# MarkFzp/Deep-Whole-Body-Control

Measured on AMD Instinct MI355X. Metric: env-steps/sec whole node, widowGo1 4096-env PPO, higher is better.
Workload: dtype f32

## Files before the change

### __graft_entry__.py

```python
import os
import subprocess
import sys

ROOT = os.path.dirname(os.path.abspath(__file__))
PKG = os.path.join(ROOT, "deep-whole-body-control_amd")
CSRC = os.path.join(PKG, "csrc")
LIB = os.path.join(PKG, "wbc_amd", "libwbc_amd.so")
SOURCES = ["wbc_sim.hip", "wbc_step_kernel.hip", "wbc_gae_kernel.hip", "wbc_policy_kernel.hip", "wbc_ppo_kernel.hip", "wbc_hist_kernel.hip", "wbc_hist_train_kernel.hip", "wbc_arm_kernel.hip", "wbc_proximity_kernel.hip", "wbc_estimator_kernel.hip", "wbc_mpc_kernel.hip", "wbc_footstep_kernel.hip", "wbc_contact_kernel.hip", "wbc_legctl_kernel.hip", "wbc_attitude_kernel.hip", "wbc_ground_kernel.hip", "wbc_slip_kernel.hip", "wbc_terrain_kernel.hip"]
for p in (PKG, os.path.join(ROOT, "oracle")):
    if p not in sys.path:
        sys.path.insert(0, p)


def _stale(target, deps):
    if not os.path.exists(target):
        return True
    t = os.path.getmtime(target)
    return any(os.path.getmtime(d) > t for d in deps)


COMMON_FLAGS = ["--offload-arch=gfx950", "-O3", "-std=c++17", "-fPIC", "-Wno-unused-result", "-fno-slp-vectorize"]
EXTRA_FLAGS = {"wbc_step_kernel.hip": ["-mllvm", "-disable-machine-licm"]}
HEADERS = ("wbc_device.h", "wbc_mlp.h", "wbc_chain_fwd.h", "wbc_ppo_chain.h", "wbc_stream_guard.h", "wbc_track.h", "wbc_stats.h", "wbc_tree.h", "wbc_urdf.h", "wbc_delassus.h", "wbc_proximity.h", "wbc_estimator.h", "wbc_mpc.h", "wbc_footstep.h", "wbc_contact.h", "wbc_legctl.h", "wbc_attitude.h", "wbc_ground.h", "wbc_slip.h")


def compile_objects(force: bool = False, extra=(), objdir=None, jobs: int = 4):
    from concurrent.futures import ThreadPoolExecutor
    objdir = objdir or os.path.join(ROOT, "build", "obj")
    os.makedirs(objdir, exist_ok=True)
    hipcc = os.environ.get("HIPCC", "/opt/rocm/bin/hipcc")
    hdrs = [os.path.join(CSRC, h) for h in HEADERS] + [os.path.join(ROOT, "include", "wbc_sim.h"), os.path.abspath(__file__)]
    todo, objs = [], []
    for src in SOURCES:
        obj = os.path.join(objdir, src.replace(".hip", ".o"))
        objs.append(obj)
        if force or _stale(obj, [os.path.join(CSRC, src)] + hdrs):
            todo.append([hipcc] + COMMON_FLAGS + EXTRA_FLAGS.get(src, []) + list(extra) + ["-c", os.path.join(CSRC, src), "-o", obj])
    with ThreadPoolExecutor(max_workers=jobs) as ex:
        list(ex.map(subprocess.check_call, todo))
    return objs


def build_product(force: bool = False) -> None:
    srcs = [os.path.join(CSRC, s) for s in SOURCES]
    deps = srcs + [os.path.join(CSRC, h) for h in HEADERS] + [os.path.join(ROOT, "include", "wbc_sim.h"), os.path.abspath(__file__)]
    if force or _stale(LIB, deps):
        objs = compile_objects(force)
        hipcc = os.environ.get("HIPCC", "/opt/rocm/bin/hipcc")
        subprocess.check_call([hipcc, "--offload-arch=gfx950", "-shared", "-fPIC", "-o", LIB] + objs)
    import wbc_amd
    from wbc_amd import native
    L = native.lib()
    missing = [s for s in native.EXPORTED_SYMBOLS if not hasattr(L, s)]
    if missing:
        raise RuntimeError(f"libwbc_amd.so lacks symbols: {missing}")


def build(force: bool = False) -> None:
    build_product(force)
    try:
        import oracle
        oracle.build(force)
    except Exception as e:
        print(f"[build] WARNING: the CPU oracle (test infrastructure) did not build: {e!r}", file=sys.stderr)


def smoke() -> None:
    import numpy as np
    import torch
    assert torch.cuda.is_available(), "smoke() needs a ROCm GPU"
    build()
    from oracle import OracleSim, default_curriculum
    from wbc_amd import abi
    from wbc_amd.config import WidowGo1RoughCfg, WidowGo1RoughCfgPPO, class_to_dict
    from wbc_amd.envs import WidowGo1
    from wbc_amd.rsl_rl.runners import OnPolicyRunner
    cfg = WidowGo1RoughCfg()
    cfg.env.num_envs = 64
    cfg.terrain.mesh_type = "plane"
    env = WidowGo1(cfg, sim_device="cuda:0", seed=3)
    o = OracleSim(env.wmodel, env.tcfg, 64, seed=3, precision="f64")
    o.set_curriculum(default_curriculum(cfg, 0))
    env.sim.reset_all()
    torch.cuda.synchronize()
    for name in abi.TENSOR_IDS:
        if name not in ("OBS_BUF",):
# ... 21 lines not shown
```

### deep-whole-body-control_amd/csrc/wbc_hist_kernel.hip

```cpp
#include <hip/hip_runtime.h>
#include "wbc_stream_guard.h"
#include <stdint.h>

#define H_T 10
#define H_NP 76
#define H_OBS 860
#define H_OFF 100
#define H_C1 30
#define H_C2 20
#define H_C3 10
#define H_OUT 20
#define H_ROWS 24
#define H_THREADS 256

struct HistParams { const float *enc_w, *enc_b, *c1_w, *c1_b, *c2_w, *c2_b, *lin_w, *lin_b; };

static __device__ __forceinline__ float elu1(float x) { return x > 0.f ? x : __expf(x) - 1.f; }

typedef float f32x4h __attribute__((ext_vector_type(4)));

static __device__ __forceinline__ void hist_latent_body(const HistParams& P, const float* __restrict__ obs, float* __restrict__ out, int rows) {
  __shared__ float b_enc[H_C1], b_c1[H_C2], b_c2[H_C3];
  __shared__ __attribute__((aligned(8))) float w_c2[H_C3][H_C2 * 2 + 2];
  __shared__ float w_lin[H_OUT][H_C1], b_lin[H_OUT];
// ... 77 lines not shown
      }
    }
    __syncthreads();
    for (int e = tid; e < H_ROWS * 3 * H_C3; e += H_THREADS) {
      const int rr = e / (3 * H_C3), rem = e - rr * (3 * H_C3), l = rem / H_C3, co = rem - l * H_C3;
      float acc = b_c2[co];
      const float* wr = w_c2[co];
#pragma unroll 4
      for (int ci = 0; ci < H_C2; ++ci) acc += h2[rr][l][ci] * wr[ci * 2] + h2[rr][l + 1][ci] * wr[ci * 2 + 1];
      h3[rr][co * 3 + l] = elu1(acc);
    }
    __syncthreads();
    for (int e = tid; e < H_ROWS * H_OUT; e += H_THREADS) {
      const int rr = e / H_OUT, j = e - rr * H_OUT;
      if (row0 + rr < rows) {
        float acc = b_lin[j];
#pragma unroll 6
        for (int i = 0; i < H_C1; ++i) acc += h3[rr][i] * w_lin[j][i];
        out[(size_t)(row0 + rr) * H_OUT + j] = elu1(acc);
      }
    }
  }
}

extern "C" __global__ void __launch_bounds__(H_THREADS, 3) wbc_hist_latent_kernel(HistParams P, const float* __restrict__ obs, float* __restrict__ out,
                                                                              int rows) {
  hist_latent_body(P, obs, out, rows);
}
extern "C" __global__ void __launch_bounds__(H_THREADS, 2) wbc_hist_latent_small_kernel(HistParams P, const float* __restrict__ obs,
                                                                                    float* __restrict__ out, int rows) {
  hist_latent_body(P, obs, out, rows);
}

extern "C" int wbc_hist_latent(const void* const* params, const float* obs, float* out, int rows, void* stream) {
  StreamDeviceGuard sdg(stream);
  if (!params || !obs || !out || rows <= 0) return -1;
  HistParams P;
  const float** dst = reinterpret_cast<const float**>(&P);
  for (int i = 0; i < 8; ++i) { if (!params[i]) return -1; dst[i] = static_cast<const float*>(params[i]); }
  const int ngroups = (rows + H_ROWS - 1) / H_ROWS;
  if (ngroups <= 512) hipLaunchKernelGGL(wbc_hist_latent_small_kernel, dim3(ngroups), dim3(H_THREADS), 0, (hipStream_t)stream, P, obs, out, rows);
  else hipLaunchKernelGGL(wbc_hist_latent_kernel, dim3(768), dim3(H_THREADS), 0, (hipStream_t)stream, P, obs, out, rows);
  return hipGetLastError() == hipSuccess ? 0 : -2;
}
```

### deep-whole-body-control_amd/wbc_amd/native.py

```python
from __future__ import annotations

import ctypes as C
import os

from . import abi

_HERE = os.path.dirname(os.path.abspath(__file__))
LIB_PATH = os.environ.get("WBC_AMD_LIB") or os.path.join(_HERE, "libwbc_amd.so")
_lib = None

c_void, c_int, c_f32p = C.c_void_p, C.c_int, C.c_void_p


class WbcError(RuntimeError):
    pass


def lib():
    global _lib
    if _lib is None:
        import torch
        if not os.path.exists(LIB_PATH):
            raise WbcError(f"{LIB_PATH} not found: build the HIP extension first "
                           f"(python -c 'import __graft_entry__ as g; g.build()')")
# ... 1 lines not shown
        L.wbc_last_error.restype = C.c_char_p
        L.wbc_sim_arena_bytes.restype = C.c_size_t
        L.wbc_sim_arena_bytes.argtypes = [c_int]
        L.wbc_sim_create.argtypes = [C.POINTER(abi.WbcModel), C.POINTER(abi.WbcTaskCfg), c_int, c_int, C.c_uint64,
                                     c_void, C.c_size_t, C.POINTER(c_void)]
        L.wbc_sim_destroy.argtypes = [c_void]
        L.wbc_sim_get_tensor.argtypes = [c_void, c_int, C.POINTER(c_void), C.POINTER(C.c_int64), C.POINTER(c_int), C.POINTER(c_int)]
        L.wbc_sim_set_env_params.argtypes = [c_void] + [c_void] * 10
        L.wbc_sim_set_heightfield.argtypes = [c_void, c_void, c_int, c_int] + [C.c_float] * 5
        L.wbc_sim_set_curriculum.argtypes = [c_void, C.POINTER(abi.WbcCurriculum)]
        L.wbc_sim_step.argtypes = [c_void, c_void, c_void]
        L.wbc_sim_step_to.argtypes = [c_void, c_void, c_void, c_void]
        L.wbc_sim_step_rollout.argtypes = [c_void, c_void, c_void, c_void, C.c_float, c_void, c_void, c_void]
        L.wbc_get_heights.argtypes = [c_void, c_int, c_void, c_int, c_void, c_void, c_int, c_int, C.c_float, C.c_float, C.c_float, c_void, c_int, c_int, c_void]
        L.wbc_sim_reset_all.argtypes = [c_void, c_void]
        L.wbc_sim_set_dof_forces.argtypes = [c_void, c_void, c_void]
        L.wbc_sim_simulate.argtypes = [c_void, c_void]
        L.wbc_sim_set_root_state.argtypes = [c_void, c_void, c_void]
        L.wbc_sim_set_dof_state.argtypes = [c_void, c_void, c_void]
        L.wbc_sim_set_root_state_indexed.argtypes = [c_void, c_void, c_void, c_int, c_void]
        L.wbc_sim_set_dof_state_indexed.argtypes = [c_void, c_void, c_void, c_int, c_void]
        for fn in ("wbc_sim_refresh_dof_state", "wbc_sim_refresh_root_state", "wbc_sim_refresh_net_contact_force",
                   "wbc_sim_refresh_force_sensor"):
            getattr(L, fn).argtypes = [c_void]
        L.wbc_sim_refresh_rigid_body_state.argtypes = [c_void, c_void]
        L.wbc_sim_get_step_counter.argtypes = [c_void, C.POINTER(C.c_int64)]
        L.wbc_sim_set_step_counter.argtypes = [c_void, C.c_int64]
        L.wbc_gae_compute.argtypes = [c_void] * 7 + [c_int, c_int, C.c_float, C.c_float, c_void]
        L.wbc_gae_normalize.argtypes = [c_void, c_void, C.c_int64, c_void]
        L.wbc_gae_workspace_doubles.argtypes = [c_int]
        L.wbc_abi_sizes.argtypes = [C.POINTER(c_int)]
        L.wbc_tensor_spec.argtypes = [c_int, C.POINTER(C.c_int64), C.POINTER(c_int), C.POINTER(c_int)]
        L.wbc_hist_latent.argtypes = [c_void, c_void, c_void, c_int, c_void]
        L.wbc_sim_arm_dynamics.argtypes = [c_void, c_void, c_void, c_void, c_void, c_void, c_void]
        L.wbc_sim_body_dynamics.argtypes = [c_void, c_void, c_void, c_void]
        L.wbc_sim_inverse_dynamics.argtypes = [c_void, c_void, c_void, c_void, c_void]
        L.wbc_sim_mass_solve.argtypes = [c_void, c_void, C.c_int64, c_int, c_void, c_int, c_void]
        L.wbc_sim_forward_dynamics.argtypes = [c_void, c_void, c_void, c_int, c_void]
        L.wbc_sim_body_accelerations.argtypes = [c_void, c_void, c_void, c_void]
        L.wbc_sim_centroidal.argtypes = [c_void] * 7
        L.wbc_sim_coriolis.argtypes = [c_void] * 5
        L.wbc_sim_momentum_observer.argtypes = [c_void, c_void, C.c_float, C.c_float, c_int, c_void, c_void]
        L.wbc_sim_proximity_pair_count.argtypes = [c_void]
        L.wbc_sim_proximity_pairs.argtypes = [c_void, c_void]
        L.wbc_sim_proximity.argtypes = [c_void] * 6 + [c_int, c_void]
        L.wbc_sim_leg_odometry.argtypes = [c_void, C.POINTER(abi.WbcEstimatorCfg)] + [c_void] * 8 + [c_int] + [c_void] * 6
        L.wbc_sim_footstep_plan.argtypes = [c_void, C.POINTER(abi.WbcFootstepCfg)] + [c_void] * 8 + [c_int] + [c_void] * 10
        L.wbc_sim_contact_detect.argtypes = ([c_void, C.POINTER(abi.WbcContactCfg)] + [c_void] * 4 + [c_int] + [c_void] * 4 + [c_int] + [c_void] * 2 +
                                             [c_int] + [c_void] * 8)
        L.wbc_sim_leg_control.argtypes = ([c_void, C.POINTER(abi.WbcLegControlCfg)] + [c_void] * 9 + [c_int, c_void, c_int, c_void, c_int] +
                                          [c_void] * 2 + [c_int] + [c_void] * 5)
        L.wbc_sim_attitude_filter.argtypes = [c_void, C.POINTER(abi.WbcAttitudeCfg)] + [c_void] * 5 + [c_int] + [c_void] * 2 + [c_int] + [c_void] * 8
        L.wbc_sim_ground_estimate.argtypes = [c_void, C.POINTER(abi.WbcGroundCfg)] + [c_void] * 6 + [c_int] * 2 + [c_void] * 9
        L.wbc_sim_slip_detect.argtypes = [c_void, C.POINTER(abi.WbcSlipCfg)] + [c_void] * 9 + [c_int] + [c_void] * 12
        L.wbc_sim_centroidal_mpc.argtypes = [c_void, C.POINTER(abi.WbcMpcCfg)] + [c_void] * 4 + [c_int] + [c_void] * 3 + [c_int] + [c_void] * 8
        L.wbc_sim_centroidal_mpc_workspace_floats.argtypes = [c_int]
        L.wbc_sim_centroidal_mpc_workspace_floats.restype = C.c_size_t
        L.wbc_sim_inverse_dynamics_derivatives.argtypes =[c_void, c_void, c_void, c_void, c_int, c_void]
        L.wbc_sim_forward_dynamics_derivatives_workspace_floats.argtypes = [c_int]
        L.wbc_sim_forward_dynamics_derivatives_workspace_floats.restype = C.c_size_t
        L.wbc_sim_forward_dynamics_derivatives.argtypes = [c_void, c_void, c_void, c_void, c_void, c_void, c_int, c_void, c_void]
        L.wbc_sim_inverse_dynamics_regressor.argtypes = [c_void, c_void, c_int, c_void, c_void, c_int, c_void]
        L.wbc_sim_forward_dynamics_sensitivity.argtypes = [c_void, c_void, c_int, c_void, c_void, c_void, c_void, c_int, c_void]
        L.wbc_sim_identification_accumulate.argtypes = [c_void, c_void, c_int, c_void, c_void, c_void, C.c_float] + [c_void] * 4 + [c_int, c_void]
        L.wbc_sim_identification_solve.argtypes = [c_void, c_int] + [c_void] * 5 + [C.c_float] + [c_void] * 6
        L.wbc_sim_constrained_dynamics_workspace_floats.argtypes = [c_int, c_int]
# ... 48 lines not shown
        L.wbc_asset_opts_default.restype = None
        L.wbc_asset_load_urdf.argtypes = [C.c_char_p, C.POINTER(abi.WbcAssetOpts), c_void, C.POINTER(c_void)]
        L.wbc_asset_dof_properties_ex.argtypes = [c_void, C.POINTER(abi.WbcDofProps)]
        L.wbc_asset_find_rigid_body.argtypes = L.wbc_asset_find_dof.argtypes = [c_void, C.c_char_p]
        L.wbc_asset_force_sensor_bodies.argtypes = [c_void, C.POINTER(C.c_int32)]
        L.wbc_ppo_sq_partials_offset.argtypes = [c_int]
        L.wbc_ppo_sq_partials_offset.restype = C.c_size_t
        L.wbc_ppo_clip_adam.argtypes = [c_void] * 4 + [C.c_float] * 7 + [c_void, c_void, c_void]
        L.wbc_ppo_clip_adam_packed.argtypes = [c_void] * 4 + [C.c_float] * 7 + [c_void, c_void, c_void, c_int, c_void]
        L.wbc_hist_train_grad.argtypes = [c_void, c_void, c_void, c_void, c_int, c_void, c_void, c_void]
        L.wbc_hist_train_workspace_floats.restype = C.c_size_t
        L.wbc_hist_clip_adam.argtypes = [c_void] * 4 + [C.c_float] * 7 + [c_int, c_void, c_void]
        L.wbc_priv_latent.argtypes = [c_void, c_void, c_void, c_int, c_void]
        L.wbc_ppo_workspace_floats.argtypes = [c_int]
        L.wbc_ppo_workspace_floats.restype = C.c_size_t
        _lib = L
    return _lib


EXPORTED_SYMBOLS = [
    "wbc_last_error", "wbc_sim_arena_bytes", "wbc_sim_create", "wbc_sim_destroy", "wbc_sim_get_tensor",
    "wbc_sim_set_env_params", "wbc_sim_set_heightfield", "wbc_sim_set_curriculum", "wbc_sim_step", "wbc_sim_step_to", "wbc_sim_step_rollout", "wbc_get_heights", "wbc_sim_reset_all",
    "wbc_sim_set_dof_forces", "wbc_sim_simulate", "wbc_sim_set_root_state", "wbc_sim_set_dof_state",
    "wbc_sim_set_root_state_indexed", "wbc_sim_set_dof_state_indexed", "wbc_sim_refresh_dof_state",
    "wbc_sim_refresh_root_state", "wbc_sim_refresh_net_contact_force", "wbc_sim_refresh_force_sensor",
    "wbc_sim_refresh_rigid_body_state", "wbc_sim_get_step_counter", "wbc_sim_set_step_counter", "wbc_gae_compute",
    "wbc_gae_normalize", "wbc_gae_workspace_doubles", "wbc_abi_sizes", "wbc_sim_episode_stats", "wbc_rollout_store", "wbc_hist_latent", "wbc_sim_arm_dynamics", "wbc_sim_body_dynamics", "wbc_sim_inverse_dynamics", "wbc_sim_mass_solve", "wbc_sim_forward_dynamics", "wbc_sim_body_accelerations", "wbc_sim_constrained_dynamics", "wbc_sim_constrained_dynamics_workspace_floats", "wbc_sim_constrained_dynamics_derivatives", "wbc_sim_constrained_dynamics_derivatives_workspace_floats", "wbc_sim_impulse_dynamics", "wbc_sim_impulse_dynamics_workspace_floats", "wbc_sim_inverse_kinematics", "wbc_sim_task_inverse_dynamics", "wbc_sim_task_inverse_dynamics_workspace_floats", "wbc_sim_task_inverse_dynamics_qp", "wbc_sim_task_inverse_dynamics_qp_workspace_floats", "wbc_sim_centroidal", "wbc_sim_inverse_dynamics_derivatives", "wbc_sim_forward_dynamics_derivatives", "wbc_sim_forward_dynamics_derivatives_workspace_floats", "wbc_sim_inverse_dynamics_regressor", "wbc_sim_forward_dynamics_sensitivity", "wbc_sim_identification_accumulate", "wbc_sim_identification_solve", "wbc_sim_proximity_pair_count", "wbc_sim_proximity_pairs", "wbc_sim_proximity", "wbc_sim_leg_odometry", "wbc_sim_footstep_plan", "wbc_sim_contact_detect", "wbc_sim_leg_control", "wbc_sim_attitude_filter", "wbc_sim_ground_estimate", "wbc_sim_slip_detect", "wbc_sim_centroidal_mpc", "wbc_sim_centroidal_mpc_workspace_floats", "wbc_policy_act", "wbc_policy_pack", "wbc_policy_pack_floats", "wbc_ppo_minibatch_grad", "wbc_ppo_minibatch_grad_packed", "wbc_ppo_pack_invalidate", "wbc_ppo_clip_adam", "wbc_ppo_clip_adam_packed", "wbc_ppo_clip_adam_workspace_floats", "wbc_ppo_grad_floats",
    "wbc_ppo_num_splits", "wbc_ppo_workspace_floats", "wbc_ppo_sq_partials_offset", "wbc_hist_train_grad", "wbc_hist_train_grad_floats",
    "wbc_hist_train_workspace_floats", "wbc_hist_clip_adam", "wbc_priv_latent", "wbc_runner_track_episodes", "wbc_sim_episode_stats_track", "wbc_tensor_spec", "wbc_policy_act_job", "wbc_sim_episode_stats_job", "wbc_side_job_run",
    "wbc_runner_track_state_floats", "wbc_asset_load", "wbc_asset_free", "wbc_asset_dof_count", "wbc_asset_rigid_body_count", "wbc_asset_dof_name",
    "wbc_asset_rigid_body_name", "wbc_asset_dof_properties", "wbc_asset_model", "wbc_asset_task_cfg", "wbc_asset_curriculum",
    "wbc_asset_opts_default", "wbc_asset_load_urdf", "wbc_asset_dof_properties_ex", "wbc_asset_find_rigid_body", "wbc_asset_find_dof",
    "wbc_asset_force_sensor_bodies"]


def check(rc: int, what: str = "") -> None:
    if rc != 0:
        raise WbcError(f"{what} failed ({rc}): {lib().wbc_last_error().decode()}")
```

### deep-whole-body-control_amd/wbc_amd/rsl_rl/algorithms/ppo.py

```python
from __future__ import annotations

import torch
import torch.nn as nn
import torch.optim as optim

from ... import collectives
from ..modules import ActorCritic
from ..storage import RolloutStorage


class PPO:
    actor_critic: ActorCritic

    def __init__(self, actor_critic, num_learning_epochs=1, num_mini_batches=1, clip_param=0.2, gamma=0.998, lam=0.95,
                 value_loss_coef=1.0, entropy_coef=0.0, learning_rate=1e-3, max_grad_norm=1.0, use_clipped_value_loss=True,
                 schedule="fixed", desired_kl=0.01, device="cpu", mixing_schedule=[0.5, 2000, 4000], torque_supervision=True,
                 torque_supervision_schedule=[0.1, 1000, 1000], adaptive_arm_gains=True, min_policy_std=None,
                 dagger_update_freq=20, priv_reg_coef_schedual=[0, 0, 0], dist_group=None):
        self.device = device
        self.desired_kl, self.schedule, self.learning_rate = desired_kl, schedule, learning_rate
        self.actor_critic = actor_critic
        self.actor_critic.to(self.device)
        self.storage = None
        self.optimizer = optim.Adam(self.actor_critic.parameters(), lr=learning_rate)
# ... 69 lines not shown
                st.privileged_observations[st.step].copy_(critic_obs)
                critic_slot = st.privileged_observations[st.step]
            else:
                critic_slot = obs_slot
            tr.observations, tr.critic_observations = obs_slot, critic_slot
        else:
            tr.observations, tr.critic_observations = obs, critic_obs
        return tr.actions

    def next_observation_slot(self):
        st = self.storage
        if st is None or st.privileged_observations is not None or not st.observations.is_cuda:
            return None
        i = st.step + 1
        return st.observations[i] if i < st.num_transitions_per_env else None

    def rollout_slots(self):
        st, tr = self.storage, self.transition
        if (st is None or st.step >= st.num_transitions_per_env or not st.rewards.is_cuda or tr.values is None or not tr.values.is_cuda
                or tr.values.dtype != torch.float32 or not tr.values.is_contiguous() or tr.values.shape != (st.num_envs, 2)):
            return None
        return tr.values, self.gamma, st.rewards[st.step], st.dones[st.step]

    def _process_env_step_fused(self, rewards, arm_rewards, dones, infos):
        st, tr = self.storage, self.transition
        if not (self.fused_rollout and st is not None and st.step < st.num_transitions_per_env and st.rewards.is_cuda
                and rewards.is_cuda and rewards.dtype == torch.float32 and arm_rewards.dtype == torch.float32
                and dones.dtype == torch.int64 and rewards.is_contiguous() and arm_rewards.is_contiguous() and dones.is_contiguous()
                and tr.values is not None and tr.values.is_cuda and tr.values.is_contiguous() and tr.values.dtype == torch.float32
                and tr.values.shape == (rewards.shape[0], 2)):
            return False
        if infos.get("rollout_stored") is not None and infos["rollout_stored"] == st.rewards[st.step].data_ptr():
            tr.rewards, tr.dones = st.rewards[st.step], st.dones[st.step]
            return True
        to = infos.get("time_outs")
        if to is not None:
            if not (to.is_cuda and to.is_contiguous() and to.dtype in (torch.bool, torch.uint8) and to.shape == rewards.shape):
                return False
        from ...native import check, lib
        i = st.step
        check(lib().wbc_rollout_store(rewards.data_ptr(), arm_rewards.data_ptr(), dones.data_ptr(), to.data_ptr() if to is not None else None,
                                      tr.values.data_ptr(), float(self.gamma), st.rewards[i].data_ptr(), st.dones[i].data_ptr(),
                                      rewards.shape[0], torch.cuda.current_stream(rewards.device).cuda_stream), "wbc_rollout_store")
        tr.rewards, tr.dones = st.rewards[i], st.dones[i]
        return True

    def process_env_step(self, rewards, arm_rewards, dones, infos):
        tr = self.transition
        if not self._process_env_step_fused(rewards, arm_rewards, dones, infos):
            tr.rewards = torch.stack([rewards.clone(), arm_rewards.clone()], dim=-1)
            tr.dones = dones
            if "time_outs" in infos:
                tr.rewards += self.gamma * torch.squeeze(tr.values * infos["time_outs"].unsqueeze(1).to(self.device), 1)
        supervised = "target_arm_torques" in infos
        if supervised:
            tr.target_arm_torques = infos["target_arm_torques"].detach()
            tr.current_arm_dof_pos = infos["current_arm_dof_pos"].detach()
            tr.current_arm_dof_vel = infos["current_arm_dof_vel"].detach()
        self.storage.add_transitions(tr, torque_supervision=supervised)
        tr.clear()
        self.actor_critic.reset(dones)

    def compute_returns(self, last_critic_obs, side_job=None):
        ac = self.actor_critic
        if self.fused_rollout and not torch.is_grad_enabled() and ac.fused_act_supported(last_critic_obs):
            last_values = ac.fused_act(last_critic_obs, side_job=side_job)[3]
# ... 15 lines not shown
        if dev.type == "cuda":
            torch.cuda.synchronize(dev)

    def _allreduce_grads(self, params):
        if self.dist_group is None:
            return
        params = [p for p in params if p.grad is not None]
        key = tuple(id(p) for p in params)
        if key not in self._buckets:
            n = sum(p.numel() for p in params)
            self._buckets[key] = torch.empty(n, dtype=params[0].dtype, device=params[0].device)
        flat = self._buckets[key]
        off = 0
        for p in params:
            flat[off:off + p.numel()].copy_(p.grad.reshape(-1))
            off += p.numel()
        collectives.all_reduce(flat, self.dist_group)
        flat.div_(self.world_size)
        off = 0
        for p in params:
            p.grad.copy_(flat[off:off + p.numel()].view_as(p.grad))
            off += p.numel()

    def _generator(self):
        if self.actor_critic.is_recurrent:
            raise NotImplementedError("recurrent policies are unreachable in the reference as well (SURVEY.md inventory #24)")
        return self.storage.mini_batch_generator(self.num_mini_batches, self.num_learning_epochs)

    def _fused_update_supported(self):
        st, ac = self.storage, self.actor_critic
        return (self.fused_update and st.observations.is_cuda and st.privileged_observations is None and not ac.is_recurrent
                and not self.torque_supervision and not (self.desired_kl is not None and self.schedule == "adaptive")
                and ac.fused_act_supported(st.observations[0]))

    def _update_fused(self):
        import ctypes as C
        from ...native import check, lib
        L, st, ac, dev = lib(), self.storage, self.actor_critic, self.storage.observations.device
        T, N = st.num_transitions_per_env, st.num_envs
        batch = T * N
        mb = batch // self.num_mini_batches
        params = ac.fused_params()
        if self._fused is None or self._fused["mb"] != mb:
            ng = L.wbc_ppo_grad_floats()
            grad = torch.zeros(ng, device=dev)
            off = 0
            for p in params:
                p.grad = grad[off:off + p.numel()].view_as(p)
                off += p.numel()
            assert off == ng - 3
            self._fused = dict(mb=mb, grad=grad, nparam=off, ws=torch.empty(L.wbc_ppo_workspace_floats(mb), device=dev),
                               hist=torch.empty(batch, 20, device=dev), m=torch.zeros(off, device=dev), v=torch.zeros(off, device=dev),
                               adam_ws=torch.empty(int(L.wbc_ppo_clip_adam_workspace_floats()), device=dev), sq_off=int(L.wbc_ppo_sq_partials_offset(mb)))
        F = self._fused
        for p, g in zip(params, torch.split(F["grad"][:F["nparam"]], [p.numel() for p in params])):
            if p.grad is None or p.grad.data_ptr() != g.data_ptr():
                p.grad = g.view_as(p)
        for p in ac.actor.history_encoder.parameters():
            p.grad = None
        table = ac.fused_param_table()
        obs = st.observations.view(batch, -1)
        with torch.inference_mode():
            if ac.actor._fused_hist_supported(obs):
                F["hist"] = ac.actor.infer_hist_latent(obs)
            else:
                for s0 in range(0, batch, 32768):
                    F["hist"][s0:s0 + 32768] = ac.actor.infer_hist_latent(obs[s0:s0 + 32768])
        flat = lambda x: x.view(batch, -1)
        actions, values, adv, returns, logp = (flat(x) for x in (st.actions, st.values, st.advantages, st.returns, st.actions_log_prob))
        value_mixing_ratio = self.get_value_mixing_ratio()
        s = self.priv_reg_coef_schedual
        priv_reg_coef = min(max((self.counter - s[2]), 0) / s[3], 1) * (s[1] - s[0]) + s[0]
        indices = torch.randperm(self.num_mini_batches * mb, requires_grad=False, device=dev)
        sums = torch.zeros(3, device=dev)
        stream = torch.cuda.current_stream(dev).cuda_stream
        vcoef = self.value_loss_coef
        steps = self._bind_adam_state(params, F)
        packed = False
        for _ in range(self.num_learning_epochs):
            for i in range(self.num_mini_batches):
                idx = indices[i * mb:(i + 1) * mb]
                check((L.wbc_ppo_minibatch_grad_packed if packed else L.wbc_ppo_minibatch_grad)(table, obs.data_ptr(), actions.data_ptr(), values.data_ptr(), adv.data_ptr(),
                                               returns.data_ptr(), logp.data_ptr(), F["hist"].data_ptr(), idx.data_ptr(), mb,
                                               float(self.clip_param), float(vcoef), float(value_mixing_ratio), float(priv_reg_coef),
                                               int(self.use_clipped_value_loss), F["ws"].data_ptr(), F["grad"].data_ptr(), sums.data_ptr(), stream),
                      "wbc_ppo_minibatch_grad")
                grad_is_fresh = True
                if self.entropy_coef != 0.0:
                    ac.std.grad.sub_(self.entropy_coef * 0.5 / ac.std.detach())
                    grad_is_fresh = False
                if self.dist_group is not None:
                    collectives.all_reduce(F["grad"][:F["nparam"]], self.dist_group)
                    grad_is_fresh = False
                if steps is None:
                    if self.world_size > 1:
                        F["grad"][:F["nparam"]].div_(self.world_size)
                    nn.utils.clip_grad_norm_(params, self.max_grad_norm)
                    self.optimizer.step()
                    packed = False
                else:
# ... 261 lines not shown
```

### deep-whole-body-control_amd/wbc_amd/rsl_rl/modules/actor_critic.py

```python
from __future__ import annotations

from typing import List, Sequence

import torch
import torch.nn as nn
from torch.distributions import Normal

_ACTIVATIONS = {"elu": nn.ELU, "selu": nn.SELU, "relu": nn.ReLU, "crelu": nn.ReLU, "lrelu": nn.LeakyReLU,
                "tanh": nn.Tanh, "sigmoid": nn.Sigmoid}


def get_activation(name: str):
    cls = _ACTIVATIONS.get(name)
    if cls is None:
        print("invalid activation function!")
        return None
    return cls()


class _SplitKLinearFn(torch.autograd.Function):
    SPLIT_K = 32
    MIN_BATCH = 4096

    @staticmethod
# ... 106 lines not shown
        self.history_encoder = StateHistoryEncoder(act, num_prop, num_hist, latent)
        if len(hidden) > 0:
            self.actor_backbone = _stack([num_prop + latent] + list(hidden), act)
            trunk = hidden[-1]
        else:
            self.actor_backbone = nn.Identity()
            trunk = num_prop + latent
        self.actor_leg_control_head = _stack([trunk] + list(leg_dims) + [n_leg], act, last_act=nn.Tanh())
        self.actor_arm_control_head = _stack([trunk] + list(arm_dims) + [n_arm], act, last_act=nn.Tanh())

    def infer_priv_latent(self, obs):
        return self.priv_encoder(obs[:, self.num_prop: self.num_prop + self.num_priv])

    def infer_hist_latent(self, obs):
        if not torch.is_grad_enabled() and self._fused_hist_supported(obs):
            return self._fused_hist_latent(obs)
        hist = obs[:, -self.num_hist * self.num_prop:]
        return self.history_encoder(hist.view(-1, self.num_hist, self.num_prop))

    def _fused_hist_supported(self, obs):
        if not (obs.is_cuda and obs.dtype == torch.float32 and obs.dim() == 2 and obs.shape[1] == 860 and obs.is_contiguous()):
            return False
        ok = self.__dict__.get("_fused_hist_ok")
        if ok is None:
            he = self.history_encoder
            ok = (self.num_hist == 10 and self.num_prop == 76 and self.num_priv == 24 and isinstance(he.activation_fn, nn.ELU)
                  and he.activation_fn.alpha == 1.0 and len(he.conv_layers) == 5
                  and tuple(he.encoder[0].weight.shape) == (30, 76) and tuple(he.conv_layers[0].weight.shape) == (20, 30, 4)
                  and tuple(he.conv_layers[2].weight.shape) == (10, 20, 2) and he.conv_layers[0].stride == (2,)
                  and he.conv_layers[2].stride == (1,) and tuple(he.linear_output[0].weight.shape) == (20, 30))
            self.__dict__["_fused_hist_ok"] = ok
        return ok

    def _fused_hist_latent(self, obs):
        import ctypes as C
        from ...native import check, lib
        he = self.history_encoder
        ps = [he.encoder[0].weight, he.encoder[0].bias, he.conv_layers[0].weight, he.conv_layers[0].bias,
              he.conv_layers[2].weight, he.conv_layers[2].bias, he.linear_output[0].weight, he.linear_output[0].bias]
        for p in ps:
            assert p.is_cuda and p.dtype == torch.float32 and p.is_contiguous()
        table = (C.c_void_p * 8)(*[p.data_ptr() for p in ps])
        out = torch.empty(obs.shape[0], 20, device=obs.device)
        check(lib().wbc_hist_latent(table, obs.data_ptr(), out.data_ptr(), obs.shape[0],
                                    torch.cuda.current_stream(obs.device).cuda_stream), "wbc_hist_latent")
        return out

    def forward(self, obs, hist_encoding=False):
        latent = self.infer_hist_latent(obs) if hist_encoding else self.infer_priv_latent(obs)
        trunk = self.actor_backbone(torch.cat([obs[:, :self.num_prop], latent], dim=1))
        leg = self.actor_leg_control_head(trunk)
        arm = self.actor_arm_control_head(trunk)
        if self.adaptive_arm_gains:
            half = self.num_arm_actions // 2
            arm = torch.cat([arm[:, :half], self.adaptive_arm_gains_scale * arm[:, half:]], dim=-1)
        return torch.cat([leg, arm], dim=-1)


class _Critic(nn.Module):
    def __init__(self, in_dim, hidden, act, leg_dims, arm_dims, num_priv, num_hist, num_prop):
        super().__init__()
        self.num_priv, self.num_hist, self.num_prop = num_priv, num_hist, num_prop
        if len(hidden) > 0:
            self.critic_backbone = _stack([in_dim] + list(hidden), act)
            trunk = hidden[-1]
        else:
            self.critic_backbone = nn.Identity()
            trunk = in_dim
        self.critic_leg_control_head = _stack([trunk] + list(leg_dims) + [1], act, act_after_last=False)
        self.critic_arm_control_head = _stack([trunk] + list(arm_dims) + [1], act, act_after_last=False)

    def forward(self, obs):
        trunk = self.critic_backbone(obs[:, :self.num_prop + self.num_priv])
        return torch.cat([self.critic_leg_control_head(trunk), self.critic_arm_control_head(trunk)], dim=-1)

# ... 151 lines not shown
```

### deep-whole-body-control_amd/wbc_amd/rsl_rl/runners/on_policy_runner.py

```python
from __future__ import annotations

import os
import statistics
import time
from collections import deque

import torch

from ... import collectives
from ..algorithms import PPO
from ..env import VecEnv
from ..modules import ActorCritic

_POLICIES = {"ActorCritic": ActorCritic}
_ALGORITHMS = {"PPO": PPO}


def _accepts(fn, name) -> bool:
    import inspect
    try:
        return name in inspect.signature(fn).parameters
    except (TypeError, ValueError):
        return False

# ... 104 lines not shown
        env, alg = self.env, self.alg
        if init_at_random_ep_len:
            env.episode_length_buf = torch.randint_like(env.episode_length_buf, high=int(env.max_episode_length))
        obs = env.get_observations()
        priv = env.get_privileged_observations()
        critic_obs = priv if priv is not None else obs
        obs, critic_obs = obs.to(self.device), critic_obs.to(self.device)
        alg.actor_critic.train()
        logging = self.log_dir is not None
        rewbuffer, armrewbuffer, lenbuffer, donebuffer = (deque(maxlen=100) for _ in range(4))
        n = env.num_envs
        cur_rew = torch.zeros(n, device=self.device)
        cur_arm = torch.zeros(n, device=self.device)
        cur_len = torch.zeros(n, device=self.device)
        ep_infos = []
        is_cuda = torch.device(self.device).type == "cuda"
        sync = (lambda: torch.cuda.synchronize(self.device)) if is_cuda else (lambda: None)
        loss_stats = dict(mean_value_loss=0., mean_surrogate_loss=0., mean_arm_torques_loss=0., value_mixing_ratio=0.,
                          torque_supervision_weight=0., mean_hist_latent_loss=0., mean_priv_reg_loss=0., priv_reg_coef=0.)
        tot_iter = self.current_learning_iteration + num_learning_iterations
        redirect_obs = hasattr(env, "set_obs_output") and hasattr(alg, "next_observation_slot") and getattr(alg, "fused_rollout", False)
        store_in_step = hasattr(env, "set_rollout_output") and hasattr(alg, "rollout_slots") and getattr(alg, "fused_rollout", False)
        tracker = None
        carry = (hasattr(env, "take_stats_job") and getattr(alg, "fused_rollout", False) and is_cuda
                 and _accepts(alg.act, "side_job") and _accepts(alg.compute_returns, "side_job"))
        if carry:
            env.defer_episode_stats = True
        try:
            for it in range(self.current_learning_iteration, tot_iter):
                env.update_command_curriculum()
                sync()
                start = time.time()
                hist_encoding = it % self.dagger_update_freq == 0
                with torch.inference_mode():
                    for _ in range(self.num_steps_per_env):
                        actions = alg.act(obs, critic_obs, hist_encoding, side_job=env.take_stats_job()) if carry else alg.act(obs, critic_obs, hist_encoding)
                        slot = alg.next_observation_slot() if redirect_obs else None
                        if slot is not None:
                            env.set_obs_output(slot)
                        if store_in_step:
                            slots = alg.rollout_slots()
                            if slots is not None:
                                env.set_rollout_output(*slots)
                        obs, priv, rewards, arm_rewards, dones, infos = env.step(actions)
                        critic_obs = priv if priv is not None else obs
                        obs, critic_obs, rewards, arm_rewards, dones = (x.to(self.device) for x in (obs, critic_obs, rewards, arm_rewards, dones))
                        alg.process_env_step(rewards, arm_rewards, dones, infos)
                        if logging:
                            if "episode" in infos:
                                ep_infos.append(infos["episode"])
                            if tracker is None:
                                tracker = _EpisodeTracker.create(env, rewards, arm_rewards, dones) or False
                            if tracker:
                                tracker.step(rewards, arm_rewards, dones)
                                continue
                            cur_rew += rewards
                            cur_arm += arm_rewards
                            cur_len += 1
                            new_ids = (dones > 0).nonzero(as_tuple=False)
                            rewbuffer.extend(cur_rew[new_ids][:, 0].cpu().numpy().tolist())
                            armrewbuffer.extend(cur_arm[new_ids][:, 0].cpu().numpy().tolist())
                            lenbuffer.extend(cur_len[new_ids][:, 0].cpu().numpy().tolist())
                            donebuffer.append(len(new_ids) / n)
                            cur_rew[new_ids] = 0
                            cur_arm[new_ids] = 0
                            cur_len[new_ids] = 0
# ... 161 lines not shown
```

### deep-whole-body-control_amd/wbc_amd/rsl_rl/storage/rollout_storage.py

```python
from __future__ import annotations

import torch

from ... import collectives


class RolloutStorage:
    class Transition:
        _FIELDS = ("observations", "critic_observations", "actions", "rewards", "dones", "values", "actions_log_prob",
                   "action_mean", "action_sigma", "hidden_states", "target_arm_torques", "current_arm_dof_pos",
                   "current_arm_dof_vel")

        def __init__(self):
            for f in self._FIELDS:
                setattr(self, f, None)

        def clear(self):
            self.__init__()

    def __init__(self, num_envs, num_transitions_per_env, obs_shape, privileged_obs_shape, actions_shape, device="cpu"):
        self.device = device
        self.obs_shape, self.privileged_obs_shape, self.actions_shape = obs_shape, privileged_obs_shape, actions_shape
        T, N = num_transitions_per_env, num_envs
        z = lambda *s, **kw: torch.zeros(T, N, *s, device=self.device, **kw)
        self.observations = z(*obs_shape)
        self.privileged_observations = z(*privileged_obs_shape) if privileged_obs_shape[0] is not None else None
        self.rewards = z(2)
        self.actions = z(*actions_shape)
        self.dones = z(1, dtype=torch.uint8)
        self.actions_log_prob, self.values, self.returns, self.advantages = z(2), z(2), z(2), z(2)
        self.mu, self.sigma = z(*actions_shape), z(*actions_shape)
        self.target_arm_torques, self.current_arm_dof_pos, self.current_arm_dof_vel = z(6), z(6), z(6)
        self.num_transitions_per_env, self.num_envs = T, N
        self.saved_hidden_states_a = self.saved_hidden_states_c = None
        self.step = 0
        self.dist_group = None
        self._gae_ws = None

    def add_transitions(self, transition: "RolloutStorage.Transition", torque_supervision):
        if self.step >= self.num_transitions_per_env:
            raise AssertionError("Rollout buffer overflow")
        i = self.step
        if transition.observations.data_ptr() != self.observations[i].data_ptr():
            self.observations[i].copy_(transition.observations)
        if self.privileged_observations is not None and \
                transition.critic_observations.data_ptr() != self.privileged_observations[i].data_ptr():
            self.privileged_observations[i].copy_(transition.critic_observations)
        def put(dst, src):
            if src.data_ptr() != dst.data_ptr() or src.dtype != dst.dtype:
                dst.copy_(src)
        put(self.actions[i], transition.actions)
        put(self.rewards[i], transition.rewards)
        put(self.dones[i], transition.dones.view(-1, 1))
        put(self.values[i], transition.values)
        put(self.actions_log_prob[i], transition.actions_log_prob)
        put(self.mu[i], transition.action_mean)
        put(self.sigma[i], transition.action_sigma)
        if torque_supervision:
            self.target_arm_torques[i].copy_(transition.target_arm_torques)
            self.current_arm_dof_pos[i].copy_(transition.current_arm_dof_pos)
            self.current_arm_dof_vel[i].copy_(transition.current_arm_dof_vel)
        self.step += 1

    def clear(self):
        self.step = 0

    def compute_returns(self, last_values, gamma, lam):
        if self.rewards.is_cuda:
            self._compute_returns_hip(last_values, gamma, lam)
        else:
            self._compute_returns_torch(last_values, gamma, lam)

    def _compute_returns_hip(self, last_values, gamma, lam):
        from ...native import check, lib
        L = lib()
        T, N = self.num_transitions_per_env, self.num_envs
        if self._gae_ws is None:
            self._gae_ws = torch.zeros(L.wbc_gae_workspace_doubles(N), dtype=torch.float64, device=self.rewards.device)
        lv = last_values.detach().to(torch.float32).contiguous()
        stream = torch.cuda.current_stream(self.rewards.device).cuda_stream
        check(L.wbc_gae_compute(self.rewards.data_ptr(), self.values.data_ptr(), self.dones.data_ptr(), lv.data_ptr(),
                                self.returns.data_ptr(), self.advantages.data_ptr(), self._gae_ws.data_ptr(), T, N,
                                float(gamma), float(lam), stream), "wbc_gae_compute")
        if self.dist_group is not None:
            collectives.all_reduce(self._gae_ws[:3], self.dist_group)
        check(L.wbc_gae_normalize(self.advantages.data_ptr(), self._gae_ws.data_ptr(), T * N * 2, stream), "wbc_gae_normalize")

    def _compute_returns_torch(self, last_values, gamma, lam):
        advantage = 0
        for step in reversed(range(self.num_transitions_per_env)):
            next_values = last_values if step == self.num_transitions_per_env - 1 else self.values[step + 1]
            not_terminal = 1.0 - self.dones[step].float()
            delta = self.rewards[step] + not_terminal * gamma * next_values - self.values[step]
            advantage = delta + not_terminal * gamma * lam * advantage
            self.returns[step] = advantage + self.values[step]
        adv = self.returns - self.values
        if self.dist_group is None:
            self.advantages = (adv - adv.mean()) / (adv.std() + 1e-8)
# ... 32 lines not shown
```

Before: 11.20 million.

## Add rollout-aware history encoder kernel reusing per-timestep encodings across overlapping windows

Adds a kernel that computes the history-encoder latent for the whole rollout by encoding each (env, timestep) proprio frame once and sharing it across the overlapping 10-step windows. Each window's start is rebuilt from the dones and the initial episode lengths. This removes the redundant per-row re-encoding of all ten history frames in the PPO update. In exchange it adds bookkeeping in storage and the runner to check the rollout was written fully in-place, and it relies on reconstructing the history-buffer reset semantics correctly, which risks mismatches against the stored observations.

```diff
diff --git a/__graft_entry__.py b/__graft_entry__.py
--- a/__graft_entry__.py
+++ b/__graft_entry__.py
@@ -51,7 +51,7 @@
     import wbc_amd
     from wbc_amd import native
     L = native.lib()
-    missing = [s for s in native.EXPORTED_SYMBOLS if not hasattr(L, s)]
+    missing = [s for s in native.EXPORTED_SYMBOLS + native.UNDECLARED_SYMBOLS if not hasattr(L, s)]
     if missing:
         raise RuntimeError(f"libwbc_amd.so lacks symbols: {missing}")
 
diff --git a/deep-whole-body-control_amd/csrc/wbc_hist_kernel.hip b/deep-whole-body-control_amd/csrc/wbc_hist_kernel.hip
--- a/deep-whole-body-control_amd/csrc/wbc_hist_kernel.hip
+++ b/deep-whole-body-control_amd/csrc/wbc_hist_kernel.hip
@@ -133,6 +133,169 @@
   hist_latent_body(P, obs, out, rows);
 }
 
+#define R_ENVS 4
+#define R_TC 40
+#define R_NF (R_TC + H_T - 1)
+#define R_ROWS 16
+#define R_THREADS 256
+#define R_ZERO (R_ENVS * R_NF)
+
+#ifdef WBC_HIST_TIMING
+__device__ long long* g_hist_dbg = nullptr;
+extern "C" int wbc_hist_set_timing_buffer(long long* buf) {
+  return hipMemcpyToSymbol(HIP_SYMBOL(g_hist_dbg), &buf, sizeof(buf)) == hipSuccess ? 0 : -2;
+}
+#define HSTAMP(i) do { if (g_hist_dbg && threadIdx.x == 0) g_hist_dbg[8 * (size_t)blockIdx.x + (i)] = clock64(); } while (0)
+#define HLAP(i) do { if (threadIdx.x == 0) { const long long now_ = clock64(); lap_[i] += now_ - last_; last_ = now_; } } while (0)
+#else
+#define HSTAMP(i)
+#define HLAP(i)
+#endif
+
+extern "C" __global__ void __launch_bounds__(R_THREADS, 4) wbc_hist_latent_rollout_kernel(HistParams P, const float* __restrict__ obs,
+    const uint8_t* __restrict__ dones, const int64_t* __restrict__ ep_len0, float* __restrict__ out, int T, int N, int env_groups) {
+  __shared__ float b_enc[H_C1], b_c1[H_C2], b_c2[H_C3];
+  __shared__ __attribute__((aligned(8))) float w_c2[H_C3][H_C2 * 2 + 2];
+  __shared__ float w_lin[H_OUT][H_C1], b_lin[H_OUT];
+  __shared__ float fc[R_ENVS * R_NF + 1][H_C1 + 1];
+  __shared__ float h2[R_ROWS][4][H_C2 + 1];
+  __shared__ float h3[R_ROWS][H_C1 + 1];
+  __shared__ short win[R_ENVS * R_TC];
+  const int tid = threadIdx.x;
+  const int lane = tid & 63, wave = tid >> 6, p = lane & 15, g = lane >> 4;
+  const int env0 = ((int)blockIdx.x % env_groups) * R_ENVS, t0 = ((int)blockIdx.x / env_groups) * R_TC;
+  HSTAMP(0);
+  const int C = min(R_TC, T - t0), nf = C + H_T - 1, npairs = R_ENVS * nf, nrows = R_ENVS * C;
+  for (int e = tid; e < H_C3 * H_C2 * 2; e += R_THREADS) w_c2[e / (H_C2 * 2)][e % (H_C2 * 2)] = P.c2_w[e];
+  for (int e = tid; e < H_OUT * H_C1; e += R_THREADS) (&w_lin[0][0])[e] = P.lin_w[e];
+  if (tid < H_C1) { b_enc[tid] = P.enc_b[tid]; fc[R_ZERO][tid] = elu1(0.f + P.enc_b[tid]); }
+  if (tid < H_C2) b_c1[tid] = P.c1_b[tid];
+  if (tid < H_C3) b_c2[tid] = P.c2_b[tid];
+  if (tid < H_OUT) b_lin[tid] = P.lin_b[tid];
+  if (tid < nrows) {
+    const int n = min(env0 + (tid & (R_ENVS - 1)), N - 1), t = t0 + tid / R_ENVS;
+    unsigned dm = 0;
+#pragma unroll
+    for (int k = 0; k < H_T + 1; ++k)
+      if (t - 1 - k >= 0 && dones[(size_t)(t - 1 - k) * N + n] != 0) dm |= 1u << k;
+    const int64_t e0 = ep_len0[n];
+    int lo = 0;
+    if (dm & 1u) lo = -1;
+    else {
+      for (int s = t - 1; s >= max(0, t - (H_T - 1)); --s) {
+        const bool refill = ((dm >> (t - s)) & 3u) != 0u || (s == 1 && e0 <= 0) || (s == 0 && e0 <= 1);
+        if (refill) { lo = s + H_T - t0; break; }
+      }
+    }
+    win[tid] = (short)lo;
+  }
+  {
+    float wA[40];
+#pragma unroll
+    for (int ks = 0; ks < 20; ++ks) {
+      const int c = g + 4 * (ks >> 2), k = 4 * c + (ks & 3);
+      wA[2 * ks] = (c < 19) ? P.enc_w[p * H_NP + k] : 0.f;
+      wA[2 * ks + 1] = (c < 19 && p + 16 < H_C1) ? P.enc_w[(p + 16) * H_NP + k] : 0.f;
+    }
+    auto fetch = [&](float4 (&a)[5], int mb) {
+      const int q = min(16 * mb + p, npairs - 1), e = q / nf, i = t0 + (q - e * nf);
+      const int n = min(env0 + e, N - 1);
+      const float* row = i < H_T ? obs + (size_t)n * H_OBS + H_OFF + i * H_NP : obs + ((size_t)(i - H_T) * N + n) * H_OBS;
+      const float4* src = reinterpret_cast<const float4*>(row);
+#pragma unroll
+      for (int j = 0; j < 5; ++j) a[j] = src[min(g + 4 * j, 18)];
+    };
+    const int nblk = (npairs + 15) / 16;
+    float4 a0[5], a1[5];
+    if (wave < nblk) fetch(a0, wave);
+    __syncthreads();
+    HSTAMP(1);
+#pragma unroll 1
+    for (int mb = wave; mb < nblk; mb += R_THREADS / 64) {
+      if (mb + R_THREADS / 64 < nblk) fetch(a1, mb + R_THREADS / 64);
+      f32x4h acc0 = {0.f, 0.f, 0.f, 0.f}, acc1 = {0.f, 0.f, 0.f, 0.f};
+#pragma unroll
+      for (int j = 0; j < 5; ++j) {
+        const float av[4] = {a0[j].x, a0[j].y, a0[j].z, a0[j].w};
+#pragma unroll
+        for (int e = 0; e < 4; ++e) {
+          acc0 = __builtin_amdgcn_mfma_f32_16x16x4f32(av[e], wA[2 * (4 * j + e)], acc0, 0, 0, 0);
+          acc1 = __builtin_amdgcn_mfma_f32_16x16x4f32(av[e], wA[2 * (4 * j + e) + 1], acc1, 0, 0, 0);
+        }
+      }
+#pragma unroll
+      for (int r4 = 0; r4 < 4; ++r4) {
+        const int q = 16 * mb + 4 * g + r4;
+        if (q < npairs) {
+          fc[q][p] = elu1(acc0[r4] + b_enc[p]);
+          if (p + 16 < H_C1) fc[q][p + 16] = elu1(acc1[r4] + b_enc[p + 16]);
+        }
+      }
+#pragma unroll
+      for (int j = 0; j < 5; ++j) a0[j] = a1[j];
+    }
+  }
+  float wB[60];
+#pragma unroll
+  for (int ci = 0; ci < H_C1; ++ci) {
+    wB[2 * ci] = P.c1_w[p * (H_C1 * 4) + ci * 4 + g];
+    wB[2 * ci + 1] = (p + 16 < H_C2) ? P.c1_w[(p + 16) * (H_C1 * 4) + ci * 4 + g] : 0.f;
+  }
+  __syncthreads();
+  HSTAMP(2);
+#ifdef WBC_HIST_TIMING
+  long long lap_[3] = {0, 0, 0}, last_ = clock64();
+#endif
+#pragma unroll 1
+  for (int row0 = 0; row0 < nrows; row0 += R_ROWS) {
+    {
+      const int q = 16 * wave + p, rq = min(row0 + (q >> 2), nrows - 1), l = q & 3;
+      const int lo = win[rq], e = rq & (R_ENVS - 1), tl = rq / R_ENVS;
+      const float* ap = &fc[lo < 0 ? R_ZERO : e * nf + max(tl + 2 * l + g, lo)][0];
+      f32x4h acc0 = {0.f, 0.f, 0.f, 0.f}, acc1 = {0.f, 0.f, 0.f, 0.f};
+#pragma unroll
+      for (int ci = 0; ci < H_C1; ++ci) {
+        const float av = ap[ci];
+        acc0 = __builtin_amdgcn_mfma_f32_16x16x4f32(av, wB[2 * ci], acc0, 0, 0, 0);
+        acc1 = __builtin_amdgcn_mfma_f32_16x16x4f32(av, wB[2 * ci + 1], acc1, 0, 0, 0);
+      }
+#pragma unroll
+      for (int r4 = 0; r4 < 4; ++r4) {
+        const int q2 = 16 * wave + 4 * g + r4, r2 = q2 >> 2, l2 = q2 & 3;
+        h2[r2][l2][p] = elu1(acc0[r4] + b_c1[p]);
+        if (p + 16 < H_C2) h2[r2][l2][p + 16] = elu1(acc1[r4] + b_c1[p + 16]);
+      }
+    }
+    __syncthreads();
+    HLAP(0);
+    for (int e = tid; e < R_ROWS * 3 * H_C3; e += R_THREADS) {
+      const int rr = e / (3 * H_C3), rem = e - rr * (3 * H_C3), l = rem / H_C3, co = rem - l * H_C3;
+      float acc = b_c2[co];
+      const float* wr = w_c2[co];
+#pragma unroll 4
+      for (int ci = 0; ci < H_C2; ++ci) acc += h2[rr][l][ci] * wr[ci * 2] + h2[rr][l + 1][ci] * wr[ci * 2 + 1];
+      h3[rr][co * 3 + l] = elu1(acc);
+    }
+    __syncthreads();
+    HLAP(1);
+    for (int e = tid; e < R_ROWS * H_OUT; e += R_THREADS) {
+      const int rr = e / H_OUT, j = e - rr * H_OUT, rq = row0 + rr;
+      const int n = env0 + (rq & (R_ENVS - 1)), t = t0 + rq / R_ENVS;
+      if (rq < nrows && n < N) {
+        float acc = b_lin[j];
+#pragma unroll 6
+        for (int i = 0; i < H_C1; ++i) acc += h3[rr][i] * w_lin[j][i];
+        out[((size_t)t * N + n) * H_OUT + j] = elu1(acc);
+      }
+    }
+    HLAP(2);
+  }
+#ifdef WBC_HIST_TIMING
+  if (g_hist_dbg && tid == 0) { for (int i = 0; i < 3; ++i) g_hist_dbg[8 * (size_t)blockIdx.x + 3 + i] = lap_[i]; }
+  HSTAMP(6);
+#endif
+}
+
 extern "C" int wbc_hist_latent(const void* const* params, const float* obs, float* out, int rows, void* stream) {
   StreamDeviceGuard sdg(stream);
   if (!params || !obs || !out || rows <= 0) return -1;
@@ -144,3 +307,17 @@
   else hipLaunchKernelGGL(wbc_hist_latent_kernel, dim3(768), dim3(H_THREADS), 0, (hipStream_t)stream, P, obs, out, rows);
   return hipGetLastError() == hipSuccess ? 0 : -2;
 }
+
+extern "C" int wbc_hist_latent_rollout(const void* const* params, const float* obs, const uint8_t* dones, const int64_t* ep_len0, float* out,
+                                       int T, int N, void* stream) {
+  StreamDeviceGuard sdg(stream);
+  if (!params || !obs || !dones || !ep_len0 || !out || T <= 0 || N <= 0 || (reinterpret_cast<uintptr_t>(obs) & 15) != 0) return -1;
+  HistParams P;
+  const float** dst = reinterpret_cast<const float**>(&P);
+  for (int i = 0; i < 8; ++i) { if (!params[i]) return -1; dst[i] = static_cast<const float*>(params[i]); }
+  const int env_groups = (N + R_ENVS - 1) / R_ENVS, chunks = (T + R_TC - 1) / R_TC;
+  if ((long long)env_groups * chunks > 0x7fffffffLL) return -1;
+  hipLaunchKernelGGL(wbc_hist_latent_rollout_kernel, dim3(env_groups * chunks), dim3(R_THREADS), 0, (hipStream_t)stream, P, obs, dones, ep_len0, out,
+                     T, N, env_groups);
+  return hipGetLastError() == hipSuccess ? 0 : -2;
+}
diff --git a/deep-whole-body-control_amd/wbc_amd/native.py b/deep-whole-body-control_amd/wbc_amd/native.py
--- a/deep-whole-body-control_amd/wbc_amd/native.py
+++ b/deep-whole-body-control_amd/wbc_amd/native.py
@@ -57,6 +57,7 @@
         L.wbc_abi_sizes.argtypes = [C.POINTER(c_int)]
         L.wbc_tensor_spec.argtypes = [c_int, C.POINTER(C.c_int64), C.POINTER(c_int), C.POINTER(c_int)]
         L.wbc_hist_latent.argtypes = [c_void, c_void, c_void, c_int, c_void]
+        L.wbc_hist_latent_rollout.argtypes = [c_void, c_void, c_void, c_void, c_void, c_int, c_int, c_void]
         L.wbc_sim_arm_dynamics.argtypes = [c_void, c_void, c_void, c_void, c_void, c_void, c_void]
         L.wbc_sim_body_dynamics.argtypes = [c_void, c_void, c_void, c_void]
         L.wbc_sim_inverse_dynamics.argtypes = [c_void, c_void, c_void, c_void, c_void]
@@ -171,6 +172,7 @@
     "wbc_asset_rigid_body_name", "wbc_asset_dof_properties", "wbc_asset_model", "wbc_asset_task_cfg", "wbc_asset_curriculum",
     "wbc_asset_opts_default", "wbc_asset_load_urdf", "wbc_asset_dof_properties_ex", "wbc_asset_find_rigid_body", "wbc_asset_find_dof",
     "wbc_asset_force_sensor_bodies"]
+UNDECLARED_SYMBOLS = ["wbc_hist_latent_rollout"]
 
 
 def check(rc: int, what: str = "") -> None:
diff --git a/deep-whole-body-control_amd/wbc_amd/rsl_rl/algorithms/ppo.py b/deep-whole-body-control_amd/wbc_amd/rsl_rl/algorithms/ppo.py
--- a/deep-whole-body-control_amd/wbc_amd/rsl_rl/algorithms/ppo.py
+++ b/deep-whole-body-control_amd/wbc_amd/rsl_rl/algorithms/ppo.py
@@ -125,6 +125,7 @@
             return False
         if infos.get("rollout_stored") is not None and infos["rollout_stored"] == st.rewards[st.step].data_ptr():
             tr.rewards, tr.dones = st.rewards[st.step], st.dones[st.step]
+            st.mark_fused_row(st.step)
             return True
         to = infos.get("time_outs")
         if to is not None:
@@ -206,6 +207,20 @@
         return (self.fused_update and st.observations.is_cuda and st.privileged_observations is None and not ac.is_recurrent
                 and not self.torque_supervision and not (self.desired_kl is not None and self.schedule == "adaptive")
                 and ac.fused_act_supported(st.observations[0]))
+
+    def storage_hist_latent(self, out=None):
+        st, ac = self.storage, self.actor_critic
+        batch = st.num_transitions_per_env * st.num_envs
+        obs = st.observations.view(batch, -1)
+        with torch.inference_mode():
+            if ac.actor._fused_hist_supported(obs):
+                if st.fused_rollout_complete():
+                    return ac.actor.infer_hist_latent_rollout(st.observations, st.dones, st.fused_ep_len0)
+                return ac.actor.infer_hist_latent(obs)
+            out = torch.empty(batch, 20, device=obs.device) if out is None else out
+            for s0 in range(0, batch, 32768):
+                out[s0:s0 + 32768] = ac.actor.infer_hist_latent(obs[s0:s0 + 32768])
+        return out
 
     def _update_fused(self):
         import ctypes as C
@@ -234,12 +249,7 @@
             p.grad = None
         table = ac.fused_param_table()
         obs = st.observations.view(batch, -1)
-        with torch.inference_mode():
-            if ac.actor._fused_hist_supported(obs):
-                F["hist"] = ac.actor.infer_hist_latent(obs)
-            else:
-                for s0 in range(0, batch, 32768):
-                    F["hist"][s0:s0 + 32768] = ac.actor.infer_hist_latent(obs[s0:s0 + 32768])
+        F["hist"] = self.storage_hist_latent(F["hist"])
         flat = lambda x: x.view(batch, -1)
         actions, values, adv, returns, logp = (flat(x) for x in (st.actions, st.values, st.advantages, st.returns, st.actions_log_prob))
         value_mixing_ratio = self.get_value_mixing_ratio()
diff --git a/deep-whole-body-control_amd/wbc_amd/rsl_rl/modules/actor_critic.py b/deep-whole-body-control_amd/wbc_amd/rsl_rl/modules/actor_critic.py
--- a/deep-whole-body-control_amd/wbc_amd/rsl_rl/modules/actor_critic.py
+++ b/deep-whole-body-control_amd/wbc_amd/rsl_rl/modules/actor_critic.py
@@ -162,15 +162,29 @@
             self.__dict__["_fused_hist_ok"] = ok
         return ok
 
-    def _fused_hist_latent(self, obs):
+    def _hist_param_table(self):
         import ctypes as C
-        from ...native import check, lib
         he = self.history_encoder
         ps = [he.encoder[0].weight, he.encoder[0].bias, he.conv_layers[0].weight, he.conv_layers[0].bias,
               he.conv_layers[2].weight, he.conv_layers[2].bias, he.linear_output[0].weight, he.linear_output[0].bias]
         for p in ps:
             assert p.is_cuda and p.dtype == torch.float32 and p.is_contiguous()
-        table = (C.c_void_p * 8)(*[p.data_ptr() for p in ps])
+        return (C.c_void_p * 8)(*[p.data_ptr() for p in ps])
+
+    def infer_hist_latent_rollout(self, obs, dones, ep_len0):
+        from ...native import check, lib
+        T, N = obs.shape[0], obs.shape[1]
+        assert not torch.is_grad_enabled() and obs.dim() == 3 and self._fused_hist_supported(obs.view(T * N, -1))
+        assert dones.is_cuda and dones.dtype == torch.uint8 and dones.is_contiguous() and dones.numel() == T * N
+        assert ep_len0.is_cuda and ep_len0.dtype == torch.int64 and ep_len0.is_contiguous() and ep_len0.shape == (N,)
+        out = torch.empty(T * N, 20, device=obs.device)
+        check(lib().wbc_hist_latent_rollout(self._hist_param_table(), obs.data_ptr(), dones.data_ptr(), ep_len0.data_ptr(), out.data_ptr(),
+                                            T, N, torch.cuda.current_stream(obs.device).cuda_stream), "wbc_hist_latent_rollout")
+        return out
+
+    def _fused_hist_latent(self, obs):
+        from ...native import check, lib
+        table = self._hist_param_table()
         out = torch.empty(obs.shape[0], 20, device=obs.device)
         check(lib().wbc_hist_latent(table, obs.data_ptr(), out.data_ptr(), obs.shape[0],
                                     torch.cuda.current_stream(obs.device).cuda_stream), "wbc_hist_latent")
diff --git a/deep-whole-body-control_amd/wbc_amd/rsl_rl/runners/on_policy_runner.py b/deep-whole-body-control_amd/wbc_amd/rsl_rl/runners/on_policy_runner.py
--- a/deep-whole-body-control_amd/wbc_amd/rsl_rl/runners/on_policy_runner.py
+++ b/deep-whole-body-control_amd/wbc_amd/rsl_rl/runners/on_policy_runner.py
@@ -160,6 +160,8 @@
                 sync()
                 start = time.time()
                 hist_encoding = it % self.dagger_update_freq == 0
+                if store_in_step and it > self.current_learning_iteration and hasattr(alg.storage, "begin_fused_rollout"):
+                    alg.storage.begin_fused_rollout(env.episode_length_buf)
                 with torch.inference_mode():
                     for _ in range(self.num_steps_per_env):
                         actions = alg.act(obs, critic_obs, hist_encoding, side_job=env.take_stats_job()) if carry else alg.act(obs, critic_obs, hist_encoding)
diff --git a/deep-whole-body-control_amd/wbc_amd/rsl_rl/storage/rollout_storage.py b/deep-whole-body-control_amd/wbc_amd/rsl_rl/storage/rollout_storage.py
--- a/deep-whole-body-control_amd/wbc_amd/rsl_rl/storage/rollout_storage.py
+++ b/deep-whole-body-control_amd/wbc_amd/rsl_rl/storage/rollout_storage.py
@@ -36,6 +36,27 @@
         self.step = 0
         self.dist_group = None
         self._gae_ws = None
+        self.fused_ep_len0 = None
+        self.fused_rows = 0
+        self._ep_len0_buf = None
+
+    def begin_fused_rollout(self, ep_len):
+        ok = (self.step == 0 and ep_len is not None and ep_len.is_cuda and ep_len.dtype == torch.int64
+              and ep_len.shape == (self.num_envs,) and ep_len.device == self.observations.device)
+        if ok:
+            if self._ep_len0_buf is None:
+                self._ep_len0_buf = torch.empty(self.num_envs, dtype=torch.int64, device=ep_len.device)
+            self._ep_len0_buf.copy_(ep_len)
+        self.fused_ep_len0, self.fused_rows = (self._ep_len0_buf if ok else None), 0
+
+    def mark_fused_row(self, i):
+        if self.fused_ep_len0 is not None and i == self.fused_rows == self.step:
+            self.fused_rows += 1
+        else:
+            self.fused_ep_len0 = None
+
+    def fused_rollout_complete(self):
+        return self.fused_ep_len0 is not None and self.fused_rows == self.step == self.num_transitions_per_env
 
     def add_transitions(self, transition: "RolloutStorage.Transition", torque_supervision):
         if self.step >= self.num_transitions_per_env:
@@ -51,6 +72,8 @@
                 dst.copy_(src)
         put(self.actions[i], transition.actions)
         put(self.rewards[i], transition.rewards)
+        if transition.dones.data_ptr() != self.dones[i].data_ptr() or self.fused_rows != i + 1:
+            self.fused_ep_len0 = None
         put(self.dones[i], transition.dones.view(-1, 1))
         put(self.values[i], transition.values)
         put(self.actions_log_prob[i], transition.actions_log_prob)
@@ -64,6 +87,7 @@
 
     def clear(self):
         self.step = 0
+        self.fused_ep_len0, self.fused_rows = None, 0
 
     def compute_returns(self, last_values, gamma, lam):
         if self.rewards.is_cuda:
```

Measured after the change: 11.13 million. Within noise of the previous version (-0.7%).
